# CapAI/ship-sim-gym

Hardware: AMD Instinct MI355X
Metric: env steps/sec (batched ShipEnv) (higher is better)
Workload: dtype f64

## Files before the change

ship_sim_gym_amd/csrc/shipsim_api.cpp:

```cpp
#include <cfloat>
#include <cmath>
#include <cstdio>
#include <cstring>
#include <algorithm>
#include <new>
#include <string>
#include <vector>

#include "shipsim.h"
#include "shipsim_internal.h"

struct ssg_handle {
    ssg_config cfg;
    ssg::DevCfg dev{};
    int n_pad = 0;
    size_t off_stats = 0, off_f64 = 0, off_i32 = 0, off_mask = 0, off_obs2 = 0, off_obsH = 0, nbytes = 0;
    size_t off_dyn_f64 = 0, off_dyn_live = 0, off_dyn_u32 = 0, off_dyn_flag = 0;
    size_t off_dyn_hash = 0, off_dyn_count = 0, off_dyn_row = 0, off_dyn_bucket = 0;
    size_t off_dyn_memo = 0, off_dyn_memo_stats = 0, off_dyn_npm = 0, off_dyn_qmap = 0;
    bool time_kernels = false;
    double t_dyn_ms = 0.0, t_step_ms = 0.0;
    unsigned long long t_steps = 0;
    unsigned long long n_classify = 0;
    int masked_resets_since_step = 0;
// ... 199 lines not shown
}

int set_ship(ssg_config *cfg, double ws, double hs, double mass)
{
    double pts[2 * SSG_SHIP_VERTS];
    std::vector<P2> v(SSG_SHIP_VERTS);
    for (int i = 0; i < SSG_SHIP_VERTS; ++i) {
        pts[2 * i] = kShipTemplate[i][0] * ws;
        pts[2 * i + 1] = kShipTemplate[i][1] * hs;
        v[i] = P2{pts[2 * i], pts[2 * i + 1]};
    }
    const double moment = moment_for_poly(mass, SSG_SHIP_VERTS, pts);
    std::vector<P2> hull = convex_hull(v);
    if ((int)hull.size() != SSG_SHIP_VERTS) return SSG_ERR_BAD_ARG;
    std::vector<Plane> pl = planes_of(hull);
    for (int i = 0; i < SSG_SHIP_VERTS; ++i) {
        cfg->ship_hull[2 * i] = hull[i].x;
        cfg->ship_hull[2 * i + 1] = hull[i].y;
        cfg->ship_normals[2 * i] = pl[i].nx;
        cfg->ship_normals[2 * i + 1] = pl[i].ny;
    }
    cfg->ship_m_inv = 1.0 / mass;
    cfg->ship_i_inv = 1.0 / moment;
    return SSG_OK;
}

int set_traffic(ssg_handle *h)
{
    static const double kTraffic[SSG_N_TRAFFIC][4] = {{100, 200, 1, 1}, {300, 200, 1.5, 2}, {400, 350, 1, 3}};
    ssg::DynCfg &d = h->dyn;
    const double mass = 1.0 / h->cfg.ship_m_inv;
    for (int k = 0; k < SSG_N_TRAFFIC; ++k) {
        ssg_config tmp = h->cfg;
        const int rc = set_ship(&tmp, kTraffic[k][2], kTraffic[k][3], mass);
        if (rc != SSG_OK) return rc;
        std::memcpy(d.thull[k], tmp.ship_hull, sizeof(d.thull[k]));
        std::memcpy(d.tnrm[k], tmp.ship_normals, sizeof(d.tnrm[k]));
        d.t_i_inv[k] = tmp.ship_i_inv;
        d.tx[k] = kTraffic[k][0];
        d.ty[k] = kTraffic[k][1];
    }
    d.t_m_inv = h->cfg.ship_m_inv;
    d.goal_m_inv = 1.0 / 1.0;
    d.goal_i_inv = 1.0 / (1.0 * 0.5 * (0.0 * 0.0 + h->cfg.goal_radius * h->cfg.goal_radius));
    d.ship_friction = 0.7;
    d.slop = 0.1;
    d.bias_coef = 1.0 - std::pow(std::pow(1.0 - 0.1, 60.0), h->cfg.dt);
    return SSG_OK;
}

void refresh_dev(ssg_handle *h)
{
    const ssg_config &c = h->cfg;
    ssg::DevCfg &d = h->dev;
    d.n_envs = c.n_envs;
    d.n_pad = h->n_pad;
    d.env_id_base = c.env_id_base;
    d.n_beams = c.n_beams;
    d.history = c.history < 2 ? c.history : 2;
    d.full_history = c.history;
    d.max_steps = c.max_steps;
    d.n_goals = c.n_goals;
    d.flags = c.flags;
    d.n_maps = h->n_maps;
    d.map_ring = c.map_ring;
    d.rudder_step = c.rudder_step;
    d.rudder_max = c.rudder_max;
    d.spread_deg = c.lidar_spread_deg;
    d.lidar_dist = c.lidar_dist;
    d.goal_r = c.goal_radius;
    d.width = c.width;
    d.height = c.height;
    d.dt = c.dt;
    d.damp = c.damping_pow_dt;
    d.spawn_x = c.spawn_x;
    d.spawn_y = c.spawn_y;
    std::memcpy(d.hull, c.ship_hull, sizeof(d.hull));
    std::memcpy(d.nrm, c.ship_normals, sizeof(d.nrm));
    d.m_inv = c.ship_m_inv;
    d.i_inv = c.ship_i_inv;
    d.force_y = c.force_y;
    d.px0 = c.thrust_px0;
    d.py0 = c.thrust_py0;
    {
        const double deg2rad = 0.017453292519943295;
        const double delta = (c.lidar_spread_deg / (double)c.n_beams) * deg2rad;
        const double phi0 = (90.0 - c.lidar_spread_deg / 2) * deg2rad;
        for (int i = 0; i < SSG_MAX_BEAMS; ++i) {
            const double phi = phi0 + delta * (double)i;
            d.beam_cos[i] = std::cos(phi);
            d.beam_sin[i] = std::sin(phi);
        }
    }
    char *base = static_cast<char *>(h->state);
    d.stats = base ? reinterpret_cast<double *>(base + h->off_stats) : nullptr;
    d.f64cols = base ? reinterpret_cast<double *>(base + h->off_f64) : nullptr;
    d.i32cols = base ? reinterpret_cast<int32_t *>(base + h->off_i32) : nullptr;
    d.mask = base ? reinterpret_cast<uint8_t *>(base + h->off_mask) : nullptr;
    d.obs2 = (base && c.history > 2) ? reinterpret_cast<double *>(base + h->off_obs2) : nullptr;
    d.obsH = (base && c.history > 2) ? reinterpret_cast<double *>(base + h->off_obsH) : nullptr;
    d.bank = h->bank;
    d.n_ships = c.n_ships;
    const bool dyn = base && c.n_ships > 1;
    d.dyn_f64 = dyn ? reinterpret_cast<double *>(base + h->off_dyn_f64) : nullptr;
    d.dyn_live = dyn ? reinterpret_cast<unsigned long long *>(base + h->off_dyn_live) : nullptr;
    d.dyn_u32 = dyn ? reinterpret_cast<uint32_t *>(base + h->off_dyn_u32) : nullptr;
    d.dyn_flag = dyn ? reinterpret_cast<uint8_t *>(base + h->off_dyn_flag) : nullptr;
    d.dyn_hash = dyn ? reinterpret_cast<unsigned long long *>(base + h->off_dyn_hash) : nullptr;
    d.dyn_count = dyn ? reinterpret_cast<unsigned *>(base + h->off_dyn_count) : nullptr;
    d.dyn_bucket = dyn ? reinterpret_cast<int32_t *>(base + h->off_dyn_bucket) : nullptr;
    d.dyn_qmap = dyn ? reinterpret_cast<int32_t *>(base + h->off_dyn_qmap) : nullptr;
    d.dyn_par = 0;
    d.dyn_row = dyn ? reinterpret_cast<double *>(base + h->off_dyn_row) : nullptr;
    const bool memo = dyn && !(c.flags & SSG_FLAG_DYN_MEMO_OFF) && c.map_ring == 0 && h->n_maps > 0 && h->n_maps <= 65536;
    d.dyn_memo = memo ? reinterpret_cast<unsigned long long *>(base + h->off_dyn_memo) : nullptr;
    d.dyn_memo_stats = dyn ? reinterpret_cast<unsigned long long *>(base + h->off_dyn_memo_stats) : nullptr;
    d.dyn_npm = memo ? reinterpret_cast<unsigned long long *>(base + h->off_dyn_npm) : nullptr;
    d.dyn_memo_gen = h->memo_gen;
    d.dyn_seq = h->dyn_seq;
    {
        unsigned long long fp = 0xcbf29ce484222325ull;
        auto eat = [&](const void *p, size_t n) { const unsigned char *b = static_cast<const unsigned char *>(p); for (size_t i = 0; i < n; ++i) fp = (fp ^ b[i]) * 0x100000001b3ull; };
        eat(h->dyn.thull, sizeof h->dyn.thull); eat(h->dyn.tnrm, sizeof h->dyn.tnrm); eat(h->dyn.tx, sizeof h->dyn.tx); eat(h->dyn.ty, sizeof h->dyn.ty);
        eat(h->dyn.t_i_inv, sizeof h->dyn.t_i_inv); eat(&h->dyn.t_m_inv, 8); eat(&h->dyn.goal_m_inv, 8); eat(&h->dyn.goal_i_inv, 8);
        eat(&h->dyn.ship_friction, 8); eat(&h->dyn.bias_coef, 8); eat(&h->dyn.slop, 8);
        eat(&c.dt, 8); eat(&c.damping_pow_dt, 8); eat(&c.goal_radius, 8); eat(&c.n_goals, 4);
        h->dyn.memo_fp = (unsigned)((fp ^ (fp >> 16) ^ (fp >> 32) ^ (fp >> 48)) & 0xFFFFu);
    }
    {
        auto radius = [](const double *hull) {
            double r2 = 0.0;
            for (int i = 0; i < SSG_SHIP_VERTS; ++i) r2 = std::max(r2, hull[2 * i] * hull[2 * i] + hull[2 * i + 1] * hull[2 * i + 1]);
            return std::sqrt(r2);
        };
        for (int k = 0; k < SSG_N_TRAFFIC; ++k) {
            const double r = radius(h->dyn.thull[k]) * 1.001 + 1.0;
            d.dyn_reach2[k] = r * r;
        }
        std::memcpy(d.thull, h->dyn.thull, sizeof(d.thull));
        std::memcpy(d.tnrm, h->dyn.tnrm, sizeof(d.tnrm));
    }
    h->dyn_queue_valid = false;
}


constexpr int kMemoGenSteps = 1 << 15;
static void memo_new_generation(ssg_handle *h)
{
    h->memo_gen += 1;
    if (h->memo_gen > 255) { h->memo_gen = 1; h->memo_clear_pending = true; }
    h->memo_steps = 0;
    h->dev.dyn_memo_gen = h->memo_gen;
}

int pick_block(int n_envs)
{
    if (const char *s = std::getenv("SSG_BLOCK")) {
        const int b = std::atoi(s);
        if (b == 64 || b == 128 || b == 256) return b;
    }
    if (n_envs <= 64 * 256) return 64;
    if (n_envs <= 128 * 256) return 128;
    return 256;
}

int refuse_capture(ssg_handle *h, void *stream, const char *what)
// ... 975 lines not shown
```

ship_sim_gym_amd/csrc/shipsim_internal.h:

```cpp
#ifndef SHIPSIM_INTERNAL_H
#define SHIPSIM_INTERNAL_H

#include <hip/hip_runtime.h>

#include <cstddef>
#include <cstdint>

#include "shipsim.h"

namespace ssg {

enum { COL_X = 0, COL_Y, COL_VX, COL_VY, COL_A, COL_W, COL_CUM, COL_LIDAR  };
enum { ICOL_RUDDER = 0, ICOL_STEP, ICOL_MAP, ICOL_EPISODE ,
       ICOL_GEN , ICOL_COUNT };

enum {
    DC_TRAFFIC = 0,
    DC_GOAL_COLS = 8,
    DC_GOALS = DC_TRAFFIC + 9 * SSG_N_TRAFFIC,
    DC_ARB = DC_GOALS + DC_GOAL_COLS * SSG_MAX_GOALS,
    kDynPairs = 54,
    kPolyPairs = 9,
    DC_PREV_GOAL = DC_ARB + 4 * kDynPairs,
    DC_TROT = DC_PREV_GOAL + 2,
    DC_COUNT = DC_TROT + 2 * SSG_N_TRAFFIC
};
enum { DU_META = 0 , DU_HASH = kDynPairs ,
       DU_COUNT = kDynPairs + kPolyPairs };

constexpr int kDynAgeBuckets = 8, kDynMapBuckets = 64, kDynBuckets = kDynAgeBuckets * kDynMapBuckets;
constexpr int kDynGrp = 48;
constexpr int kDynPad = kDynMapBuckets * kDynGrp;
constexpr int kDynBucketStride = 32;
constexpr int kDynCountWords = kDynBuckets * kDynBucketStride;
__host__ __device__ __forceinline__ constexpr int dyn_counter_word(unsigned bucket) { return (int)bucket * kDynBucketStride; }
__host__ __device__ __forceinline__ unsigned dyn_bucket_of(int age, int map_id)
{
    const unsigned agek = (unsigned)(age < kDynAgeBuckets - 1 ? (age < 0 ? 0 : age) : kDynAgeBuckets - 1);
    return ((unsigned)map_id & (unsigned)(kDynMapBuckets - 1)) * (unsigned)kDynAgeBuckets + agek;
}
constexpr int kDynRow = 80, kDynRowTraffic = 48;
constexpr int kMemoEntries = 1 << 14;
enum { ME_TAG = 0, ME_READY, ME_BORN, ME_PAD, ME_KEY };
constexpr int kMemoArbIn = 4, kMemoArbOut = 8, kMemoAged = 4, kMemoArbWords = 6 ;
constexpr int kMemoKeyShips = 2, kMemoKeyGoals = kMemoKeyShips + 28 , kMemoKeyArbs = kMemoKeyGoals + 8 * SSG_MAX_GOALS;
constexpr int kMemoKeyWords = kMemoKeyArbs + kMemoArbIn * kMemoArbWords;
constexpr int ME_VAL = ME_KEY + kMemoKeyWords;
constexpr int kMemoValShipWords = 12 ;
constexpr int kMemoValShips = 2, kMemoValGoals = kMemoValShips + kMemoValShipWords * SSG_N_TRAFFIC, kMemoValArbs = kMemoValGoals + 8 * SSG_MAX_GOALS;
constexpr int kMemoValAged = kMemoValArbs + kMemoArbOut * kMemoArbWords;
constexpr int kMemoValWords = kMemoValAged + kMemoAged;
constexpr int kMemoStride = ME_VAL + kMemoValWords;
static_assert(kMemoKeyGoals % 2 == 0 && kMemoKeyArbs % 2 == 0 && kMemoValGoals % 2 == 0 && kMemoValArbs % 2 == 0 && kMemoValAged % 2 == 0, "even sections");
constexpr int kMemoProbes = 4;
constexpr int kNpmEntries = 1 << 14, kNpmProbes = 2;
enum { NE_KEY = 4, NE_VAL = NE_KEY + 6, kNpmStride = NE_VAL + 12 };
constexpr int kMemoStatSlots = 256, kMemoStatWords = 16;
static_assert(ME_KEY % 2 == 0 && ME_VAL % 2 == 0 && kMemoStride % 2 == 0, "16-byte loads of key and value");
constexpr int kPadEnvs = 256;
constexpr int kStatsSlots = 256;
constexpr int kStatsDoubles = 4 * kStatsSlots;

struct DevCfg {
    int n_envs, n_pad;
    long long env_id_base;
    int n_beams, history , max_steps, n_goals;
    int full_history;
    double *obs2;
    double *obsH;
    unsigned flags;
    int n_maps;
    int map_ring;
    int rudder_step, rudder_max;
    double spread_deg, lidar_dist, goal_r, width, height, dt, damp, spawn_x, spawn_y;
    double hull[2 * SSG_SHIP_VERTS], nrm[2 * SSG_SHIP_VERTS];
    double m_inv, i_inv, force_y, px0, py0;
    double beam_cos[SSG_MAX_BEAMS], beam_sin[SSG_MAX_BEAMS];
    double *f64cols;
    int32_t *i32cols;
    uint8_t *mask;
    double *stats;
    const double *bank;
    unsigned long long *dbg;
    double *term_obs;
    int n_ships;
    double *dyn_f64;
    uint32_t *dyn_u32;
    unsigned long long *dyn_live;
    uint8_t *dyn_flag;
    unsigned long long *dyn_hash;
    int32_t *dyn_bucket;
    unsigned *dyn_count;
    int32_t *dyn_qmap;
    int dyn_par;
    double dyn_reach2[SSG_N_TRAFFIC];
    double thull[SSG_N_TRAFFIC][2 * SSG_SHIP_VERTS], tnrm[SSG_N_TRAFFIC][2 * SSG_SHIP_VERTS];
    double *dyn_row;
    unsigned long long *dyn_memo;
    unsigned long long *dyn_memo_stats;
    unsigned long long *dyn_npm;
    unsigned long long dyn_seq;
    unsigned dyn_memo_gen;
};

struct DynCfg {
    double thull[SSG_N_TRAFFIC][2 * SSG_SHIP_VERTS], tnrm[SSG_N_TRAFFIC][2 * SSG_SHIP_VERTS];
    double tx[SSG_N_TRAFFIC], ty[SSG_N_TRAFFIC], t_i_inv[SSG_N_TRAFFIC], t_m_inv;
    double goal_m_inv, goal_i_inv;
    double ship_friction;
    double bias_coef, slop;
    unsigned bank_epoch;
    int stop_after;
    unsigned memo_fp;
};

hipError_t launch_step(const DevCfg &c, int epw, bool lds, size_t lds_bytes, const int32_t *actions_kn, int K, double *obs,
                       double *reward, uint8_t *done, uint8_t *flags, long long traj, hipStream_t stream);
size_t step_lds_bytes(int n_beams, int block, bool lds_bank, int n_maps, bool dyn );
hipError_t prepare_step(const DevCfg &c, int block, bool lds, size_t lds_bytes);
hipError_t launch_reset(const DevCfg &c, const uint8_t *mask, const int32_t *map_ids, double *obs, hipStream_t stream);
hipError_t launch_dyn_step(const DevCfg &c, const DynCfg &d, bool classify, hipStream_t stream);
hipError_t prepare_dyn(const DevCfg &c);
hipError_t launch_dyn_invalidate(const DevCfg &c, const uint8_t *mask, hipStream_t stream);
hipError_t launch_dyn_reset(const DevCfg &c, const DynCfg &d, const uint8_t *mask, const int32_t *map_ids, double *obs, bool append, hipStream_t stream);
hipError_t launch_render(const DevCfg &c, const DynCfg &d, int e, int width, int height, uint8_t *rgb, unsigned flags,
                         hipStream_t stream);
hipError_t launch_calib_copy8(const double *src, double *dst, size_t n, hipStream_t stream);
hipError_t launch_clock_probe(unsigned long long *out, int n_blocks, int iters, hipStream_t stream);
hipError_t launch_remap_map_ids(const DevCfg &c, hipStream_t stream);
hipError_t launch_history_shift(const DevCfg &c, const uint8_t *done, double *obs, hipStream_t stream);
hipError_t launch_generate_bank(uint64_t seed, int n_maps, int n_goals, double width, double height, double width_frac,
                                double spawn_x, double spawn_y, double *bank, double *raw, hipStream_t stream);
hipError_t launch_refill_worlds(const DevCfg &c, uint64_t seed, double width_frac, unsigned long long *queue, unsigned *count,
                                double *bank, double *raw, hipStream_t stream);
hipError_t launch_fill_actions(uint64_t seed, uint64_t step0, int K, long long env_base, int n, int32_t *out,
                               hipStream_t stream);
size_t policy_lds_bytes(const ssg_policy &p);
hipError_t prepare_policy();
hipError_t launch_policy_act(const ssg_policy &p, int n, long long env_base, const double *obs, const float *uniform, uint64_t seed,
                             int64_t step, int32_t *act, float *logp, float *value, float *x, hipStream_t stream);
constexpr size_t kPpoStatsOff = 0, kPpoSlotsOff = 256;
constexpr int kPpoMaxGrid = 512;
inline int ppo_gae_blocks(long long N) { return (int)((N + 255) / 256); }
int ppo_packed_len(const ssg_policy &p);
int ppo_grid(long long M);
size_t ppo_grad_lds_bytes(const ssg_policy &p);
hipError_t prepare_ppo();
hipError_t launch_ppo_gae(const ssg_ppo_hparams &hp, int K, int N, const double *rew, const uint8_t *done, const float *val,
                          const float *last_val, float *adv, float *ret, void *ws, hipStream_t stream);
hipError_t launch_ppo_grad(const ssg_policy &p, const ssg_ppo_hparams &hp, long long n_samples, const float *x, const int32_t *act,
                           const float *logp, const float *adv, const float *ret, const int64_t *idx, long long M, void *ws,
                           float *grad_out, float *stats_out, float *adam_mv, int64_t step, hipStream_t stream);
hipError_t launch_ppo_adam(const ssg_policy &p, const ssg_ppo_hparams &hp, const float *grad, float *adam_mv, int64_t step,
                           hipStream_t stream);

#ifdef __HIPCC__
__device__ __forceinline__ void philox_round(uint32_t (&ctr)[4], const uint32_t (&key)[2])
{
    const uint64_t p0 = (uint64_t)0xD2511F53u * ctr[0];
    const uint64_t p1 = (uint64_t)0xCD9E8D57u * ctr[2];
    const uint32_t n0 = (uint32_t)(p1 >> 32) ^ ctr[1] ^ key[0];
    const uint32_t n1 = (uint32_t)p1;
    const uint32_t n2 = (uint32_t)(p0 >> 32) ^ ctr[3] ^ key[1];
    const uint32_t n3 = (uint32_t)p0;
    ctr[0] = n0; ctr[1] = n1; ctr[2] = n2; ctr[3] = n3;
}

__device__ __forceinline__ int reset_env(const DevCfg &c, const int e, const int32_t *__restrict__ map_ids, double *__restrict__ obs)
{
    const size_t np = (size_t)c.n_pad;
    int m;
    const int started = c.i32cols[ICOL_EPISODE * np + e];
    if (map_ids) m = (int)((unsigned)map_ids[e] % (unsigned)c.n_maps);
    else if (c.map_ring > 0) m = e * c.map_ring + started % c.map_ring;
    else m = (int)((c.env_id_base + (long long)e) % (long long)c.n_maps);
    c.i32cols[ICOL_EPISODE * np + e] = started + 1;
    const double *rec = c.bank + (size_t)m * SSG_MAP_STRIDE;
    c.f64cols[COL_X * np + e] = c.spawn_x;
    c.f64cols[COL_Y * np + e] = c.spawn_y;
    c.f64cols[COL_VX * np + e] = 0.0;
    c.f64cols[COL_VY * np + e] = 0.0;
    c.f64cols[COL_A * np + e] = 0.0;
    c.f64cols[COL_W * np + e] = 0.0;
    c.f64cols[COL_CUM * np + e] = 0.0;
    for (int i = 0; i < c.n_beams; ++i) c.f64cols[(COL_LIDAR + i) * np + e] = -1.0;
// ... 53 lines not shown
```

ship_sim_gym_amd/csrc/shipsim_kernels.hip:

```cpp
#include <hip/hip_runtime.h>

#include <cfloat>
#include <cstdint>
#include <type_traits>

#include "shipsim.h"
#include "shipsim_internal.h"

namespace ssg {

__device__ __forceinline__ double *lds_base()
{
    extern __shared__ double s_lds[];
    return s_lds;
}

__device__ __forceinline__ double dmin(double a, double b) { return __builtin_fmin(a, b); }
__device__ __forceinline__ double dmax(double a, double b) { return __builtin_fmax(a, b); }

__device__ __forceinline__ double obs_fma(double a, double b, double c)
{
#ifndef SSG_NO_LIDAR_FMA
    return __builtin_fma(a, b, c);
#else
// ... 513 lines not shown
    constexpr int FF = 6 + NB;
    constexpr int DH = H2 ? 2 * FF : FF;
    constexpr int CS = ObsTile<NB>::CS, CP = ObsTile<NB>::CP;
    int lds_at[CP], gl_at[CP];
    unsigned okmask = 0;
    int ln_ = lane;
    asm volatile("" : "+v"(ln_));
#pragma unroll
    for (int jj = 0; jj < CP; ++jj) {
        lds_at[jj] = ot.lds_of(jj, ln_);
        gl_at[jj] = ot.row_of(jj, ln_) * DH + ot.col_of(jj, ln_);
        okmask |= (ot.row_of(jj, ln_) < rows_live) ? (1u << jj) : 0u;
        if constexpr (!ObsTile<NB>::kOnTheFly) asm volatile("" : "+v"(lds_at[jj]), "+v"(gl_at[jj]));
    }
    asm volatile("" : "+v"(okmask));
#pragma unroll
    for (int pi = P_BEGIN; pi < P_END; ++pi) {
        const int p0 = pi * CP;
        if (p0 >= DH) break;
        const int cpp = (DH - p0 < CP) ? (DH - p0) : CP;
#pragma unroll
        for (int cc = 0; cc < CP; ++cc) {
            if (cc < cpp) colbuf[cc * CS + lane] = val(p0 + cc);
        }
        if (cpp == CP) {
#pragma unroll
            for (int jj = 0; jj < CP; ++jj) {
                const double v = colbuf[lds_at[jj]];
                if ((okmask >> jj) & 1u) st_out(&obase[(unsigned)(gl_at[jj] + p0)], v);
            }
        } else {
            int ln = lane;
            asm volatile("" : "+v"(ln));
#pragma unroll
            for (int jj = 0; jj < CP; ++jj) {
                if (jj < cpp) {
                    const int t = ln + 64 * jj;
                    const int r = t / cpp, cc = t - r * cpp;
                    const double v = colbuf[cc * CS + r];
                    if (r < rows_live) st_out(&obase[(unsigned)(r * DH + p0 + cc)], v);
                }
            }
        }
        __builtin_amdgcn_sched_barrier(0);
    }
}

template <int NB, bool H2, int C_BEGIN, int C_END, class Val>
__device__ __forceinline__ void write_obs_pairs(double *buf , const Val &val ,
                                                double *__restrict__ obase, const int rows_live, const int lane)
{
    constexpr int FF = 6 + NB;
    constexpr int DH = H2 ? 2 * FF : FF;
    static_assert(C_BEGIN % 2 == 0 && C_END % 2 == 0 && DH % 2 == 0 && NB >= 8, "pairs of columns; 64 x 8 doubles of buffer");
    int ln = lane;
    asm volatile("" : "+v"(ln));
    const int wsw = (ln >> 2) & 3;
#pragma unroll
    for (int c0 = C_BEGIN; c0 < C_END; c0 += 8) {
        constexpr int kMax = 4;
        const int np = ((C_END - c0) / 2 < kMax) ? (C_END - c0) / 2 : kMax;
#pragma unroll
        for (int q = 0; q < kMax; ++q)
            if (q < np) *reinterpret_cast<double2 *>(buf + ln * 8 + 2 * (q ^ wsw)) = make_double2(val(c0 + 2 * q), val(c0 + 2 * q + 1));
#pragma unroll
        for (int jj = 0; jj < kMax; ++jj) {
            if (jj < np) {
                const int pidx = ln + 64 * jj;
                const int r = (np == 4) ? (pidx >> 2) : (np == 2) ? (pidx >> 1) : (np == 1) ? pidx : pidx / 3;
                const int q = pidx - r * np;
                const double2 v = *reinterpret_cast<const double2 *>(buf + r * 8 + 2 * (q ^ ((r >> 2) & 3)));
                if (r < rows_live) *reinterpret_cast<double2 *>(&obase[(unsigned)(r * DH + c0 + 2 * q)]) = v;
            }
        }
        __builtin_amdgcn_sched_barrier(0);
    }
}

template <bool LDS_BANK>
__device__ __forceinline__ bool bank_narrowphase(const DevCfg &c, const double *shiptab, const double x, const double y,
                                                 const double ca, const double sa, const int rec_off, const bool live,
                                                 const int lane, const int only ,
                                                 const double *hL = nullptr ,
                                                 const int ld = 0)
{
    const int wq = lane / 5, wi = lane - 5 * wq;
    const double w_hx = shiptab[0 * 8 + wi], w_hy = shiptab[1 * 8 + wi];
    const double w_nx = shiptab[2 * 8 + wi], w_ny = shiptab[3 * 8 + wi];
    double swx[SSG_SHIP_VERTS], swy[SSG_SHIP_VERTS], sbl, sbr, sbb, sbt;
    ship_world(shiptab, ca, sa, x, y, swx, swy, sbl, sbr, sbb, sbt);
    bool colliding = false;
    unsigned nearbits = 0;
    int cnts = 0;
#pragma unroll
    for (int s = 0; s < 2; ++s) {
        double al, ab, ar, at, cn;
        if constexpr (LDS_BANK) {
            const double2 lb = bank_at2<LDS_BANK>(c, rec_off + SSG_MAP_OFF_AABB + 4 * s + 0);
            const double2 rt = bank_at2<LDS_BANK>(c, rec_off + SSG_MAP_OFF_AABB + 4 * s + 2);
            al = lb.x; ab = lb.y; ar = rt.x; at = rt.y;
            cn = bank_at<LDS_BANK>(c, rec_off + SSG_MAP_OFF_COUNTS + s);
        } else {
            al = hL[(SSG_MAP_OFF_AABB + 4 * s + 0) * ld]; ab = hL[(SSG_MAP_OFF_AABB + 4 * s + 1) * ld];
            ar = hL[(SSG_MAP_OFF_AABB + 4 * s + 2) * ld]; at = hL[(SSG_MAP_OFF_AABB + 4 * s + 3) * ld];
            cn = hL[(SSG_MAP_OFF_COUNTS + s) * ld];
        }
        const bool near = live & !SSG_ABL(4) & ((only < 0) | (only == s)) & (sbl <= ar) & (al <= sbr);
        (void)ab; (void)at; (void)sbb; (void)sbt;
        nearbits |= near ? (1u << s) : 0u;
        cnts |= ((int)cn) << (8 * s);
    }
#pragma unroll
    for (int s = 0; s < 2; ++s) {
        const bool near_s = (nearbits >> s) & 1u;
        if (!__any(near_s)) continue;
        const int cnt = (cnts >> (8 * s)) & 0xFF;
        bool sep = false;
        if constexpr (LDS_BANK) {
            for (int j = 0; __any(near_s & !sep & (j < cnt)); ++j) {
                if (near_s & !sep & (j < cnt)) {
                    const int q = rec_off + SSG_MAP_OFF_PLANES + s * (SSG_MAX_HULL * SSG_PLANE_DOUBLES) + SSG_PLANE_DOUBLES * j;
                    const double2 nn = bank_at2<LDS_BANK>(c, q + 2);
                    const double nx = nn.x, ny = nn.y;
                    const double v0n = bank_at<LDS_BANK>(c, q + 4);
                    bool allfront = true;
#pragma unroll
                    for (int i = 0; i < SSG_SHIP_VERTS; ++i) allfront = allfront & ((nx * swx[i] + ny * swy[i]) > v0n);
                    sep = allfront;
                }
            }
        } else {
            constexpr int kNpChunk = 4;
            for (int j0 = 0; __any(near_s & !sep & (j0 < cnt)); j0 += kNpChunk) {
                if (near_s & !sep & (j0 < cnt)) {
                    double nx[kNpChunk], ny[kNpChunk], v0n[kNpChunk];
#pragma unroll
                    for (int u = 0; u < kNpChunk; ++u) {
                        const int j = (j0 + u < SSG_MAX_HULL) ? j0 + u : 0;
                        const int q = rec_off + SSG_MAP_OFF_PLANES + s * (SSG_MAX_HULL * SSG_PLANE_DOUBLES) + SSG_PLANE_DOUBLES * j;
                        const double2 nn = bank_at2<LDS_BANK>(c, q + 2);
                        nx[u] = nn.x; ny[u] = nn.y;
                        v0n[u] = bank_at<LDS_BANK>(c, q + 4);
                    }
#pragma unroll
                    for (int u = 0; u < kNpChunk; ++u) {
                        bool allfront = j0 + u < cnt;
#pragma unroll
                        for (int i = 0; i < SSG_SHIP_VERTS; ++i) allfront = allfront & ((nx[u] * swx[i] + ny[u] * swy[i]) > v0n[u]);
                        sep = sep | allfront;
                    }
                }
            }
        }
        nearbits = sep ? (nearbits & ~(1u << s)) : nearbits;
    }
    unsigned long long todo = __ballot(nearbits != 0u);
    while (todo) {
        const int src = __ffsll((long long)todo) - 1;
        todo &= todo - 1;
        const double bx = readlane_f64(x, src), by = readlane_f64(y, src);
        const double bca = readlane_f64(ca, src), bsa = readlane_f64(sa, src);
        const int boff = __builtin_amdgcn_readlane(rec_off, src);
        const unsigned bnear = (unsigned)__builtin_amdgcn_readlane((int)nearbits, src);
        const int bcnts = __builtin_amdgcn_readlane(cnts, src);
        const double svx = bca * w_hx + (-bsa) * w_hy + bx, svy = bsa * w_hx + bca * w_hy + by;
        const double snx_ = bca * w_nx + (-bsa) * w_ny, sny_ = bsa * w_nx + bca * w_ny;
        const double off_i = snx_ * svx + sny_ * svy;
        bool col = false;
#pragma unroll
        for (int s = 0; s < 2; ++s) {
            if (!(bnear & (1u << s))) continue;
            const int cnt = (bcnts >> (8 * s)) & 0xFF;
            const bool valid = (lane < 60) & (wq < cnt);
// ... 200 lines not shown
            }
            const double *tt = traffictab + kk * 32;
            bool sep;
            {
                const double nx = bca * w_nx + (-bsa) * w_ny, ny = bsa * w_nx + bca * w_ny;
                const double vx_ = bca * w_hx + (-bsa) * w_hy + bx, vy_ = bsa * w_hx + bca * w_hy + by;
                const double off = nx * vx_ + ny * vy_;
                double mn = INFINITY;
#pragma unroll
                for (int j = 0; j < SSG_SHIP_VERTS; ++j) {
                    const double gx = tt[0 * 8 + j], gy = tt[1 * 8 + j];
                    const double qx = tca * gx + (-tsa) * gy + tx, qy = tsa * gx + tca * gy + ty;
                    mn = dmin(mn, nx * qx + ny * qy);
                }
                sep = mn > off;
            }
            {
                const double lnx = tt[2 * 8 + wi], lny = tt[3 * 8 + wi], lvx = tt[0 * 8 + wi], lvy = tt[1 * 8 + wi];
                const double nx = tca * lnx + (-tsa) * lny, ny = tsa * lnx + tca * lny;
                const double vx_ = tca * lvx + (-tsa) * lvy + tx, vy_ = tsa * lvx + tca * lvy + ty;
                const double off = nx * vx_ + ny * vy_;
                double mn = INFINITY;
#pragma unroll
                for (int j = 0; j < SSG_SHIP_VERTS; ++j) {
                    const double hx = shiptab[0 * 8 + j], hy = shiptab[1 * 8 + j];
                    const double qx = bca * hx + (-bsa) * hy + bx, qy = bsa * hx + bca * hy + by;
                    mn = dmin(mn, nx * qx + ny * qy);
                }
                sep |= mn > off;
            }
            const unsigned long long ms = __ballot(valid & sep);
            const bool separated = ((ms >> (5 * wq)) & 31ull) != 0ull;
            if (valid & (wi == 0) & !separated) atomicOr(&tw[src], 1u);
        }
        gtraf[part * EPW + tl] = (tw[lane] != 0u) ? 1u : 0u;
    };
    auto traffic_hit = [&](int) -> unsigned { return gtraf[tl] | gtraf[EPW + tl]; };
    if (role < 2) {
        unsigned short *queue = reinterpret_cast<unsigned short *>(tile_base + 2 * lds_res_bytes(NB) + role * lds_queue_bytes(NB0));
        const int b_first = role ? NB0 : 0, b_count = role ? (NB - NB0) : NB0;
        double ca, sa, cx, cy;
        int map_id;
        double tpre[DYN ? 4 * SSG_N_TRAFFIC : 1] = {};
        {
            const double x = colX[el_], y = colY[el_], ang = colA[el_];
            map_id = colMap[el_];
            if constexpr (!LDS_BANK) load_hdr_lidar(map_id * SSG_MAP_STRIDE);
            { const double2 sc = sincos_call(ang); sa = sc.x; ca = sc.y; }
            if (role == 0) { pose[2 * EPW + tl] = ca; pose[3 * EPW + tl] = sa; }
            flush_tables();
            if (LDS_BANK) __builtin_amdgcn_s_waitcnt(0);
            __syncthreads();
            SSG_STAMP(9);
            if constexpr (DYN) {
                {
                    const double *tcol = c.dyn_f64 + (size_t)DC_TRAFFIC * np, *trot = c.dyn_f64 + (size_t)DC_TROT * np;
#pragma unroll
                    for (int kk = 0; kk < SSG_N_TRAFFIC; ++kk) {
                        if ((kk == 0) != (role == 0)) continue;
                        tpre[4 * kk + 0] = tcol[(size_t)(9 * kk) * np + el_]; tpre[4 * kk + 1] = tcol[(size_t)(9 * kk + 1) * np + el_];
                        tpre[4 * kk + 2] = trot[(size_t)(2 * kk) * np + el_]; tpre[4 * kk + 3] = trot[(size_t)(2 * kk + 1) * np + el_];
                    }
                }
            }
            double swx[SSG_SHIP_VERTS], swy[SSG_SHIP_VERTS], bl, br, bb, bt;
            ship_world(shiptab, ca, sa, x, y, swx, swy, bl, br, bb, bt);
            cx = x + (br - bl) / 2;
            cy = y + (bt - bb) / 2;
        }
        lidar_query<NB, LDS_BANK, EXACT>(c, reinterpret_cast<unsigned long long *>(tile_base), queue, beamtab, b_first, b_count,
                                         cx, cy, ca, sa, map_id * SSG_MAP_STRIDE, live, lane, hL, EPW);
        if (K == 1) query_done();
        for (int k = 0; k < K; ++k) {
            if constexpr (NR == 4) wait_pose(k);
            if constexpr (DYN) {
#pragma unroll
                for (int i = 0; i < 4 * SSG_N_TRAFFIC; ++i) asm volatile("" : "+v"(tpre[i]));
            }
            SSG_STAMP_K(0);
            double nca = 0.0, nsa = 0.0, ncx = 0.0, ncy = 0.0, npx = 0.0, npy = 0.0;
            int nmap = 0;
            if constexpr (NR == 4) {
                nca = pose[2 * EPW + tl]; nsa = pose[3 * EPW + tl];
                ncx = pose[4 * EPW + tl]; ncy = pose[5 * EPW + tl];
                npx = pose[0 * EPW + tl]; npy = pose[1 * EPW + tl];
                nmap = posem[tl];
                ack_pose();
                reinterpret_cast<unsigned short *>(gres)[2 * ((k & 1) * EPW + tl) + role] =
                        bank_narrowphase<LDS_BANK>(c, shiptab, npx, npy, nca, nsa, nmap * SSG_MAP_STRIDE, live, lane, role, hL, EPW) ? 1 : 0;
            }
            SSG_STAMP_K(4);
            if constexpr (DYN) {
                static_assert(lds_queue_bytes(1) >= 64 * 2 + 64 * 4, "lidar-lo's pair queue holds ship 0's pair queue and hit words");
                unsigned short *tq1 = reinterpret_cast<unsigned short *>(traffic_scratch0 + (tl >> 6) * kTrafficScratchBytes);
                if (role == 0) traffic_collide(std::integral_constant<int, 0>{}, std::integral_constant<int, 1>{}, tpre, npx, npy, nca, nsa, 0,
                                               queue, reinterpret_cast<unsigned *>(queue + 64));
                else traffic_collide(std::integral_constant<int, 1>{}, std::integral_constant<int, SSG_N_TRAFFIC>{}, tpre, npx, npy, nca, nsa, 1,
                                     tq1, reinterpret_cast<unsigned *>(tq1 + 64 * SSG_N_TRAFFIC));
            }

            SSG_STAMP_K(3);
            tile_barrier(k);
            SSG_STAMP_K(1);
            if constexpr (NR == 6) {
                if (k + 1 < K) {
                    nca = pose[2 * EPW + tl]; nsa = pose[3 * EPW + tl];
                    ncx = pose[4 * EPW + tl]; ncy = pose[5 * EPW + tl];
                    nmap = posem[tl];
                    ack_pose();
                }
            }
            if (k + 1 < K) {
                const bool rs = auto_reset & ((gres[(k & 1) * EPW + tl] | (gdone[(k & 1) * EPW + tl] & 1u) | (DYN ? traffic_hit(k) : 0u)) != 0u);
                ca = rs ? 1.0 : nca; sa = rs ? 0.0 : nsa;
                cx = rs ? shiptab[0 * 8 + 6] : ncx; cy = rs ? shiptab[1 * 8 + 6] : ncy;
                map_id = rs ? next_map(c, nmap, el_) : nmap;
                if constexpr (!LDS_BANK) {
                    if (rs) load_hdr_lidar(map_id * SSG_MAP_STRIDE);
                }
                lidar_query<NB, LDS_BANK, EXACT>(c, reinterpret_cast<unsigned long long *>(tile_base + ((k + 1) & 1) * lds_res_bytes(NB)),
                                                 queue, beamtab, b_first, b_count, cx, cy, ca, sa, map_id * SSG_MAP_STRIDE, live, lane, hL, EPW);
                if (k + 1 == K - 1) query_done();
            }
            SSG_STAMP_K(2);
        }
        if (K == 1 && live) {
            const bool rs = auto_reset & ((gres[tl] | (gdone[tl] & 1u) | (DYN ? traffic_hit(0) : 0u)) != 0u);
            const unsigned long long *rk = reinterpret_cast<const unsigned long long *>(tile_base);
            for (int kb = 0; kb < b_count; ++kb) {
                const int i = b_first + kb;
                const unsigned long long key = rk[i * 64 + lane];
                const double hitd = __longlong_as_double((long long)(key & 0x7FFFFFFFFFFFFFFFull));
                if (rs | (key != kLidarMiss)) st_out(&colLid[(size_t)i * np + el_], rs ? -1.0 : hitd);
            }
        }
        SSG_STAMP(10);
        SSG_STAMP_FLUSH(3);
        SSG_CLOCK_END();
        return;
    }

    if constexpr (NR == 6) {
        if (role >= 4) {
            const int h = role - 4;
            int map0 = colMap[el_];
            if constexpr (!LDS_BANK) load_hdr_lidar(map0 * SSG_MAP_STRIDE);
            asm volatile("" : "+v"(map0));
            flush_tables();
            if (LDS_BANK) __builtin_amdgcn_s_waitcnt(0);
            __syncthreads();
            SSG_STAMP(9);
            for (int k = 0; k < K; ++k) {
                wait_pose(k);
                SSG_STAMP_K(0);
                const double nca = pose[2 * EPW + tl], nsa = pose[3 * EPW + tl];
                const double npx = pose[0 * EPW + tl], npy = pose[1 * EPW + tl];
                const int nmap = posem[tl];
                ack_pose();
                reinterpret_cast<unsigned short *>(gres)[2 * ((k & 1) * EPW + tl) + h] =
                        bank_narrowphase<LDS_BANK>(c, shiptab, npx, npy, nca, nsa, nmap * SSG_MAP_STRIDE, live, lane, h, hL, EPW) ? 1 : 0;
                SSG_STAMP_K(1);
                tile_barrier(k);
                SSG_STAMP_K(2);
                if constexpr (!LDS_BANK) {
                    if (k + 1 < K) {
                        const bool rs = auto_reset & ((gres[(k & 1) * EPW + tl] | (gdone[(k & 1) * EPW + tl] & 1u)) != 0u);
                        if (rs) load_hdr_lidar(next_map(c, nmap, el_) * SSG_MAP_STRIDE);
                    }
                }
            }
            SSG_STAMP(10);
            SSG_STAMP_FLUSH(5);
            return;
        }
    }

    const int wq = lane / 5, wi = lane - 5 * wq;

    if (role == 2) {
        constexpr int F = 6 + NB;
        double pv[F];
        double ogp[DYN ? 2 * SSG_MAX_GOALS : 1];
        unsigned gm_pre = 0u;
        {
            const int el = el_;
            const double x0 = colX[el], y0 = colY[el], a0 = colA[el];
            const int rud0 = colRud[el], map0 = colMap[el];
            const unsigned gm0 = c.mask[el];
#pragma unroll
            for (int i = 0; i < NB; ++i) pv[6 + i] = colLid[(size_t)i * np + el];
            pv[0] = x0; pv[1] = y0; pv[2] = (double)rud0; pv[3] = a0;
            if constexpr (DYN) {
                pv[4] = c.dyn_f64[(size_t)(DC_PREV_GOAL + 0) * np + el];
                pv[5] = c.dyn_f64[(size_t)(DC_PREV_GOAL + 1) * np + el];
            }
#pragma unroll
            for (int i = 0; i < 4; ++i) asm volatile("" : "+v"(pv[i]));
#pragma unroll
            for (int i = 0; i < NB; ++i) asm volatile("" : "+v"(pv[6 + i]));
            if constexpr (DYN) asm volatile("" : "+v"(pv[4]), "+v"(pv[5]));
            int map0_ = map0; unsigned gm0_ = gm0;
            asm volatile("" : "+v"(map0_), "+v"(gm0_));
            gm_pre = gm0_;
            flush_tables();
            if (LDS_BANK) __builtin_amdgcn_s_waitcnt(0);
            __syncthreads();
            SSG_STAMP(9);
            if constexpr (!DYN)
                nearest_goal<LDS_BANK, false>(c, map0_ * SSG_MAP_STRIDE + SSG_MAP_OFF_GOALS, gm0_, pv[0], pv[1], pv[4], pv[5], hG, EPW);
        }
        const bool hist2 = c.history >= 2;
        ObsTile<NB> ot;
        ot.init(lane);
        constexpr int kObsPasses = (2 * F + ObsTile<NB>::CP - 1) / ObsTile<NB>::CP;
        constexpr bool kPairs = (NB >= 8) && (NB % 2 == 0);
        constexpr bool kSplitOk = kPairs || (F % ObsTile<NB>::CP) == 0;
        const bool split_last = kSplitOk && hist2 && c.history == 2 && !SSG_ABL(7);
        for (int k = 0; k < K; ++k) {
            const bool early = split_last && (k == K - 1);
            if constexpr (kSplitOk) {
                if (early) {
                    int tw = __builtin_amdgcn_readfirstlane(tl >> 6);
                    int te0 = blockIdx.x * EPW + 64 * tw;
                    asm volatile("" : "+s"(tw), "+s"(te0));
                    double *colbuf = reinterpret_cast<double *>(scratch0 + tw * lds_tile_bytes(NB) + ((k + 1) & 1) * lds_res_bytes(NB));
                    double *__restrict__ ob = obs + ((size_t)te0 + (size_t)k * (size_t)traj) * (size_t)(2 * F);
                    if constexpr (kPairs)
                        write_obs_pairs<NB, true, 0, F>(colbuf, [&](int j) -> double { return pv[(j < F) ? j : 0]; }, ob, min(64, c.n_envs - te0), lane);
                    else
                        write_obs_tile<NB, true, 0, F / ObsTile<NB>::CP>(ot, colbuf, [&](int j) -> double { return pv[(j < F) ? j : 0]; }, ob,
                                                                        min(64, c.n_envs - te0), lane);
                }
            }
            if constexpr (DYN) {
#pragma unroll
                for (int g = 0; g < SSG_MAX_GOALS; ++g) {
                    const bool listed = g < c.n_goals;
                    ogp[2 * g] = listed ? goal_at<LDS_BANK, DYN>(c, el_, g, 0) : 0.0;
                    ogp[2 * g + 1] = listed ? goal_at<LDS_BANK, DYN>(c, el_, g, 1) : 0.0;
                }
            }
            wait_pose(k);
            if constexpr (DYN) {
// ... 198 lines not shown
    int act_next = actions_kn[el_];
    double gpre[DYN ? 2 * SSG_MAX_GOALS : 1];
    unsigned dflag = 0;
    unsigned long long dlive = 0ull;
    auto ask_goals = [&]() {
#pragma unroll
        for (int g = 0; g < SSG_MAX_GOALS; ++g) {
            const bool listed = g < c.n_goals;
            gpre[2 * g] = listed ? goal_at<LDS_BANK, DYN>(c, el_, g, 0) : 0.0;
            gpre[2 * g + 1] = listed ? goal_at<LDS_BANK, DYN>(c, el_, g, 1) : 0.0;
        }
        dflag = c.dyn_flag[el_];
        dlive = c.dyn_live[el_];
    };
    auto have_goals = [&]() {
#pragma unroll
        for (int g = 0; g < 2 * SSG_MAX_GOALS; ++g) asm volatile("" : "+v"(gpre[g]));
        asm volatile("" : "+v"(dflag), "+v"(dlive));
    };
    asm volatile("" : "+v"(x), "+v"(y), "+v"(vx), "+v"(vy), "+v"(ang), "+v"(w), "+v"(cum));
    asm volatile("" : "+v"(gm), "+v"(map_id), "+v"(rudder), "+v"(steps), "+v"(episodes), "+v"(act_next));
    flush_tables();
    if (LDS_BANK) __builtin_amdgcn_s_waitcnt(0);
    __syncthreads();
    SSG_STAMP(9);
    if constexpr (DYN) ask_goals();
    const double w_hx = shiptab[0 * 8 + wi], w_hy = shiptab[1 * 8 + wi];
    const double w_nx = shiptab[2 * 8 + wi], w_ny = shiptab[3 * 8 + wi];
#ifdef SSG_PRIO
    __builtin_amdgcn_s_setprio(SSG_PRIO);
#endif

    bool q_need = false;
    long long st_ret = 0;
    int st_len = 0, st_eps = 0, st_goals = 0;
    unsigned q_bucket = 0, q_arrival = 0;
    for (int k = 0; k < K; ++k) {
#ifdef SSG_STAMPS_ITER
    if (k < 8) SSG_STAMP(k);
    if (k == K - 1) SSG_STAMP(11);
    if (k == 12) SSG_STAMP(12);
    if (k == 16) SSG_STAMP(13);
#else
    SSG_STAMP_K(0);
#endif
    int el = el_;
    asm volatile("" : "+v"(el));
    const int act = act_next;
    const int rec_off = map_id * SSG_MAP_STRIDE;
    const int goff = DYN ? el_ : rec_off + SSG_MAP_OFF_GOALS;

    double fx = 0.0, fy = 0.0, tq = 0.0;
    {
        const double ca0 = pose[2 * EPW + tl], sa0 = pose[3 * EPW + tl];
        const double px = (gm & 0x80u) ? (0.0 - (double)rudder) : c.px0;
        const double py = c.py0;
        const double fwx = (-sa0) * c.force_y, fwy = ca0 * c.force_y;
        const double pwx = ca0 * px + (-sa0) * py + x, pwy = sa0 * px + ca0 * py + y;
        const double rx = pwx - x, ry = pwy - y;
        const bool thrust = act == 0;
        fx = thrust ? fwx : 0.0;
        fy = thrust ? fwy : 0.0;
        tq = thrust ? (rx * fwy - ry * fwx) : 0.0;
    }
    if (act == 1 || act == 2) {
        rudder += (act == 1) ? -c.rudder_step : c.rudder_step;
        rudder = max(-c.rudder_max, min(c.rudder_max, rudder));
        gm |= 0x80u;
    }

    x = x + vx * c.dt;
    y = y + vy * c.dt;
    ang = ang + w * c.dt;
    vx = vx * c.damp + (fx * c.m_inv) * c.dt;
    vy = vy * c.damp + (fy * c.m_inv) * c.dt;
    w = w * c.damp + tq * c.i_inv * c.dt;
    double sa, ca;
    if constexpr (DYN) {
        sincos_body(ang, &sa, &ca);
    } else {
        const double2 sc = sincos_call(ang); sa = sc.x; ca = sc.y;
    }

    double sbl, sbr, sbb, sbt;
    {
        double swx[SSG_SHIP_VERTS], swy[SSG_SHIP_VERTS];
        ship_world(shiptab, ca, sa, x, y, swx, swy, sbl, sbr, sbb, sbt);
    }
    while (__hip_atomic_load(&sync_ack[tile], __ATOMIC_ACQUIRE, __HIP_MEMORY_SCOPE_WORKGROUP) != (unsigned)(NR - 1) * (unsigned)k)
        __builtin_amdgcn_s_sleep(1);
    pose[0 * EPW + tl] = x; pose[1 * EPW + tl] = y; pose[2 * EPW + tl] = ca; pose[3 * EPW + tl] = sa;
    pose[4 * EPW + tl] = x + (sbr - sbl) / 2;
    pose[5 * EPW + tl] = y + (sbt - sbb) / 2;
    pose[6 * EPW + tl] = ang;
    posem[tl] = map_id;
    poser[tl] = rudder;
    SSG_STAMP_K(1);
    if (lane == 0) __hip_atomic_store(&sync_ready[tile], (unsigned)(k + 1), __ATOMIC_RELEASE, __HIP_MEMORY_SCOPE_WORKGROUP);
    SSG_STAMP_K(2);
    if constexpr (DYN) have_goals();

    const bool oob_x = (x < 0.0) | (x > c.width);
    const bool oob_y = (y < 0.0) | (y > c.height);

    bool goal_reached;
    {
        const double w_px = shiptab[4 * 8 + wi], w_py = shiptab[5 * 8 + wi];
        unsigned short *gq = reinterpret_cast<unsigned short *>(goal_scratch0 + (tl >> 6) * kGoalScratchBytes);
        unsigned *gw = reinterpret_cast<unsigned *>(gq + 64 * SSG_MAX_GOALS);
        gw[lane] = 0u;
        int n_pairs = 0;
        auto near_test = [&](int g, double gx, double gy) {
            const double r = c.goal_r;
            const bool near = live & !SSG_ABL(5) & (bool)((gm >> g) & 1u) & ((gx - r) <= sbr) & (sbl <= (gx + r)) &
                              ((gy - r) <= sbt) & (sbb <= (gy + r));
            const unsigned long long m = __ballot(near);
            const int pos = n_pairs + (int)__builtin_amdgcn_mbcnt_hi((unsigned)(m >> 32), __builtin_amdgcn_mbcnt_lo((unsigned)m, 0u));
            if (near) gq[pos] = (unsigned short)(lane | (g << 6));
            n_pairs += __popcll(m);
        };
        if constexpr (!LDS_BANK && !DYN) {
#pragma unroll
            for (int g = 0; g < SSG_MAX_GOALS; ++g)
                if (g < c.n_goals) near_test(g, hG[(2 * g) * EPW], hG[(2 * g + 1) * EPW]);
        } else if constexpr (DYN) {
#pragma unroll
            for (int g = 0; g < SSG_MAX_GOALS; ++g)
                if (g < c.n_goals) near_test(g, gpre[2 * g], gpre[2 * g + 1]);
        } else {
            for (int g = 0; g < c.n_goals; ++g) near_test(g, goal_at<LDS_BANK, DYN>(c, goff, g, 0), goal_at<LDS_BANK, DYN>(c, goff, g, 1));
        }
        for (int base = 0; base < n_pairs; base += 12) {
            const int p = base + wq;
            const bool valid = (lane < 60) & (p < n_pairs);
            const unsigned code = gq[valid ? p : 0];
            const int src = code & 63, g = code >> 6;
            const double bx = __shfl(x, src), by = __shfl(y, src), bca = __shfl(ca, src), bsa = __shfl(sa, src);
            const int boff = __shfl(goff, src);
            double gx, gy;
            if constexpr (!LDS_BANK && !DYN) { gx = hG[(2 * g) * EPW - lane + src]; gy = hG[(2 * g + 1) * EPW - lane + src]; }
            else if constexpr (DYN) {
                (void)boff;
                gx = __shfl(gpre[0], src); gy = __shfl(gpre[1], src);
#pragma unroll
                for (int h = 1; h < SSG_MAX_GOALS; ++h) {
                    const double hx = __shfl(gpre[2 * h], src), hy = __shfl(gpre[2 * h + 1], src);
                    gx = (g == h) ? hx : gx; gy = (g == h) ? hy : gy;
                }
            }
            else { gx = goal_at<LDS_BANK, DYN>(c, boff, g, 0); gy = goal_at<LDS_BANK, DYN>(c, boff, g, 1); }
            const double v1x = bca * w_hx + (-bsa) * w_hy + bx, v1y = bsa * w_hx + bca * w_hy + by;
            const double v0x = bca * w_px + (-bsa) * w_py + bx, v0y = bsa * w_px + bca * w_py + by;
            const double snx_ = bca * w_nx + (-bsa) * w_ny, sny_ = bsa * w_nx + bca * w_ny;
            const bool out_i = (snx_ * (gx - v1x) + sny_ * (gy - v1y)) > 0.0;
            const double dx = v0x - v1x, dy = v0y - v1y;
            const double tt = dmax(0.0, dmin((dx * (gx - v1x) + dy * (gy - v1y)) / (dx * dx + dy * dy), 1.0));
            const double qx = v1x + dx * tt, qy = v1y + dy * tt;
            const double ex_ = gx - qx, ey_ = gy - qy;
            const double dist = sqrt(ex_ * ex_ + ey_ * ey_);
            double md = dist;
#pragma unroll
            for (int kk = 1; kk < SSG_SHIP_VERTS; ++kk) {
                int o = wi + kk;
                o = (o >= SSG_SHIP_VERTS) ? o - SSG_SHIP_VERTS : o;
                md = dmin(md, __shfl(dist, 5 * wq + o));
            }
            const unsigned long long mo = __ballot(valid & out_i);
            const bool outside = ((mo >> (5 * wq)) & 31ull) != 0ull;
            const double sd = outside ? md : -md;
            if (valid & (wi == 0) & (sd <= c.goal_r)) atomicOr(&gw[src], 1u << g);
        }
        const unsigned gotmask = gw[lane];
        goal_reached = gotmask != 0u;
        gm &= ~gotmask;
    }
    steps += 1;
    const int steps_after = steps;
    const unsigned alive = gm & ((1u << c.n_goals) - 1u);
    const bool done3 = (alive == 0u) | oob_x | oob_y | (steps >= c.max_steps);
    gdone[(k & 1) * EPW + tl] = (done3 ? 1u : 0u) | (goal_reached ? 4u : 0u) | ((oob_x | oob_y) ? 8u : 0u) |
                                ((steps_after >= c.max_steps) ? 16u : 0u) | ((alive == 0u) ? 32u : 0u) | (alive << 8);
    if (k + 1 < K) act_next = actions_kn[(size_t)(k + 1) * c.n_envs + el];

    SSG_STAMP_K(3);
    tile_barrier(k);
    SSG_STAMP_K(4);

    bool colliding = gres[(k & 1) * EPW + tl] != 0u;
    if constexpr (DYN) {
        colliding |= traffic_hit(k) != 0u;
    }

    double rew = goal_reached ? 1.0 : ((oob_x | oob_y) ? -1.0 : -0.01);
    if ((c.flags & SSG_FLAG_FIX_COLLISION_REWARD) && (colliding & !goal_reached)) rew = -1.0;
    cum += rew;

    const bool done = colliding | done3;
    const bool do_reset = done & auto_reset;
// ... 344 lines not shown
```

Before: 13.44 billion.

## Replace per-step hull transform with rotated-box goal broadphase and move centre calc

The main stepping path no longer transforms every hull vertex to world space to get the ship's bounding box. The goal near-test now uses a conservative rotated-box bound built from hull extents precomputed on the host, with a small padding term for rounding. The centre pose values consumed by the other roles are now derived from the box that narrowphase already computes. This cuts per-lane arithmetic on the critical path before the pose handoff, at the cost of a slightly looser goal broadphase and a new dependency on the narrowphase output. The added SSG_ABL(10) term in the near-test is unrelated to speed.

```diff
diff --git a/ship_sim_gym_amd/csrc/shipsim_api.cpp b/ship_sim_gym_amd/csrc/shipsim_api.cpp
--- a/ship_sim_gym_amd/csrc/shipsim_api.cpp
+++ b/ship_sim_gym_amd/csrc/shipsim_api.cpp
@@ -305,6 +305,19 @@
     d.force_y = c.force_y;
     d.px0 = c.thrust_px0;
     d.py0 = c.thrust_py0;
+    {
+        double lx = INFINITY, hx = -INFINITY, ly = INFINITY, hy = -INFINITY, ax = 0.0, ay = 0.0;
+        for (int i = 0; i < SSG_SHIP_VERTS; ++i) {
+            lx = std::min(lx, c.ship_hull[2 * i]); hx = std::max(hx, c.ship_hull[2 * i]);
+            ly = std::min(ly, c.ship_hull[2 * i + 1]); hy = std::max(hy, c.ship_hull[2 * i + 1]);
+            ax = std::max(ax, std::fabs(c.ship_hull[2 * i])); ay = std::max(ay, std::fabs(c.ship_hull[2 * i + 1]));
+        }
+        d.gbox_cx = (lx + hx) / 2;
+        d.gbox_cy = (ly + hy) / 2;
+        d.gbox_hx = (hx - lx) / 2;
+        d.gbox_hy = (hy - ly) / 2;
+        d.gbox_pad = c.goal_radius + std::ldexp(ax + ay + c.goal_radius, -36);
+    }
     {
         const double deg2rad = 0.017453292519943295;
         const double delta = (c.lidar_spread_deg / (double)c.n_beams) * deg2rad;
diff --git a/ship_sim_gym_amd/csrc/shipsim_internal.h b/ship_sim_gym_amd/csrc/shipsim_internal.h
--- a/ship_sim_gym_amd/csrc/shipsim_internal.h
+++ b/ship_sim_gym_amd/csrc/shipsim_internal.h
@@ -60,6 +60,8 @@
 constexpr int kPadEnvs = 256;
 constexpr int kStatsSlots = 256;
 constexpr int kStatsDoubles = 4 * kStatsSlots;
+
+constexpr double kGoalBoxRel = 0x1p-40;
 
 struct DevCfg {
     int n_envs, n_pad;
@@ -101,6 +103,7 @@
     unsigned long long *dyn_npm;
     unsigned long long dyn_seq;
     unsigned dyn_memo_gen;
+    double gbox_cx, gbox_cy, gbox_hx, gbox_hy, gbox_pad;
 };
 
 struct DynCfg {
diff --git a/ship_sim_gym_amd/csrc/shipsim_kernels.hip b/ship_sim_gym_amd/csrc/shipsim_kernels.hip
--- a/ship_sim_gym_amd/csrc/shipsim_kernels.hip
+++ b/ship_sim_gym_amd/csrc/shipsim_kernels.hip
@@ -619,13 +619,14 @@
                                                  const double ca, const double sa, const int rec_off, const bool live,
                                                  const int lane, const int only ,
                                                  const double *hL = nullptr ,
-                                                 const int ld = 0)
+                                                 const int ld = 0, double *box = nullptr )
 {
     const int wq = lane / 5, wi = lane - 5 * wq;
     const double w_hx = shiptab[0 * 8 + wi], w_hy = shiptab[1 * 8 + wi];
     const double w_nx = shiptab[2 * 8 + wi], w_ny = shiptab[3 * 8 + wi];
     double swx[SSG_SHIP_VERTS], swy[SSG_SHIP_VERTS], sbl, sbr, sbb, sbt;
     ship_world(shiptab, ca, sa, x, y, swx, swy, sbl, sbr, sbb, sbt);
+    if (box) { box[0] = sbl; box[1] = sbr; box[2] = sbb; box[3] = sbt; }
     bool colliding = false;
     unsigned nearbits = 0;
     int cnts = 0;
@@ -992,12 +993,13 @@
             int nmap = 0;
             if constexpr (NR == 4) {
                 nca = pose[2 * EPW + tl]; nsa = pose[3 * EPW + tl];
-                ncx = pose[4 * EPW + tl]; ncy = pose[5 * EPW + tl];
                 npx = pose[0 * EPW + tl]; npy = pose[1 * EPW + tl];
                 nmap = posem[tl];
                 ack_pose();
+                double sbox[4];
                 reinterpret_cast<unsigned short *>(gres)[2 * ((k & 1) * EPW + tl) + role] =
-                        bank_narrowphase<LDS_BANK>(c, shiptab, npx, npy, nca, nsa, nmap * SSG_MAP_STRIDE, live, lane, role, hL, EPW) ? 1 : 0;
+                        bank_narrowphase<LDS_BANK>(c, shiptab, npx, npy, nca, nsa, nmap * SSG_MAP_STRIDE, live, lane, role, hL, EPW, sbox) ? 1 : 0;
+                if (k + 1 < K) { ncx = npx + (sbox[1] - sbox[0]) / 2; ncy = npy + (sbox[3] - sbox[2]) / 2; }
             }
             SSG_STAMP_K(4);
             if constexpr (DYN) {
@@ -1067,8 +1069,13 @@
                 const double npx = pose[0 * EPW + tl], npy = pose[1 * EPW + tl];
                 const int nmap = posem[tl];
                 ack_pose();
+                double sbox[4];
                 reinterpret_cast<unsigned short *>(gres)[2 * ((k & 1) * EPW + tl) + h] =
-                        bank_narrowphase<LDS_BANK>(c, shiptab, npx, npy, nca, nsa, nmap * SSG_MAP_STRIDE, live, lane, h, hL, EPW) ? 1 : 0;
+                        bank_narrowphase<LDS_BANK>(c, shiptab, npx, npy, nca, nsa, nmap * SSG_MAP_STRIDE, live, lane, h, hL, EPW, sbox) ? 1 : 0;
+                if (h == 0 && k + 1 < K) {
+                    pose[4 * EPW + tl] = npx + (sbox[1] - sbox[0]) / 2;
+                    pose[5 * EPW + tl] = npy + (sbox[3] - sbox[2]) / 2;
+                }
                 SSG_STAMP_K(1);
                 tile_barrier(k);
                 SSG_STAMP_K(2);
@@ -1433,16 +1440,9 @@
         const double2 sc = sincos_call(ang); sa = sc.x; ca = sc.y;
     }
 
-    double sbl, sbr, sbb, sbt;
-    {
-        double swx[SSG_SHIP_VERTS], swy[SSG_SHIP_VERTS];
-        ship_world(shiptab, ca, sa, x, y, swx, swy, sbl, sbr, sbb, sbt);
-    }
     while (__hip_atomic_load(&sync_ack[tile], __ATOMIC_ACQUIRE, __HIP_MEMORY_SCOPE_WORKGROUP) != (unsigned)(NR - 1) * (unsigned)k)
         __builtin_amdgcn_s_sleep(1);
     pose[0 * EPW + tl] = x; pose[1 * EPW + tl] = y; pose[2 * EPW + tl] = ca; pose[3 * EPW + tl] = sa;
-    pose[4 * EPW + tl] = x + (sbr - sbl) / 2;
-    pose[5 * EPW + tl] = y + (sbt - sbb) / 2;
     pose[6 * EPW + tl] = ang;
     posem[tl] = map_id;
     poser[tl] = rudder;
@@ -1456,15 +1456,18 @@
 
     bool goal_reached;
     {
+        const double bcx = x + (ca * c.gbox_cx + (-sa) * c.gbox_cy);
+        const double bcy = y + (sa * c.gbox_cx + ca * c.gbox_cy);
+        const double bwx = fabs(ca) * c.gbox_hx + fabs(sa) * c.gbox_hy + (c.gbox_pad + kGoalBoxRel * fabs(x));
+        const double bwy = fabs(sa) * c.gbox_hx + fabs(ca) * c.gbox_hy + (c.gbox_pad + kGoalBoxRel * fabs(y));
         const double w_px = shiptab[4 * 8 + wi], w_py = shiptab[5 * 8 + wi];
         unsigned short *gq = reinterpret_cast<unsigned short *>(goal_scratch0 + (tl >> 6) * kGoalScratchBytes);
         unsigned *gw = reinterpret_cast<unsigned *>(gq + 64 * SSG_MAX_GOALS);
         gw[lane] = 0u;
         int n_pairs = 0;
         auto near_test = [&](int g, double gx, double gy) {
-            const double r = c.goal_r;
-            const bool near = live & !SSG_ABL(5) & (bool)((gm >> g) & 1u) & ((gx - r) <= sbr) & (sbl <= (gx + r)) &
-                              ((gy - r) <= sbt) & (sbb <= (gy + r));
+            const bool in_x = fabs(gx - bcx) <= bwx, in_y = fabs(gy - bcy) <= bwy;
+            const bool near = live & !SSG_ABL(5) & !SSG_ABL(10) & (bool)((gm >> g) & 1u) & in_x & in_y;
             const unsigned long long m = __ballot(near);
             const int pos = n_pairs + (int)__builtin_amdgcn_mbcnt_hi((unsigned)(m >> 32), __builtin_amdgcn_mbcnt_lo((unsigned)m, 0u));
             if (near) gq[pos] = (unsigned short)(lane | (g << 6));
```

New measurement: 13.62 billion, median of 6. +1.3%, better.
